# aagbotemi/zk-cryptography

Hardware: AMD Instinct MI355X
Metric: field-evals/s (sumcheck 2^24) + MSM points/s (KZG 2^20) per BASELINE.json; value = the sumcheck prover's field-evals/s, the MSM half is under "msm" (higher is better)
Workload: dtype u32; 1 GPU; 24-var multilinear sumcheck prover (poly_sum + prove), BLS12-381 Fr; field=BLS12-381 Fr (255-bit Montgomery, 8 x u32 limbs); G1 over Fq (381-bit), evals_per_gpu=16777216, exchanges_per_prove=0

## Files before the change

### zk-cryptography_amd/csrc/multifold_kernels.hpp

```cpp
#pragma once
#include "sumcheck_kernels.hpp"
#include "wide_acc.hpp"

namespace zk {

constexpr int MF_MAX_LOGK = 8;
constexpr int MF_CAP_LOGK = 9;

static __global__ __launch_bounds__(MLE_BLOCK) void chunk_sums_kernel(const uint64_t* __restrict__ in, uint32_t chunk,
                                                                      uint64_t* __restrict__ partials) {
    __shared__ Fr red[MLE_BLOCK / 64];
    const uint64_t* base = in + 4 * (size_t)blockIdx.x * chunk;
    Fr s = Fr::zero();
    for (uint32_t j = threadIdx.x; j < chunk; j += 4 * MLE_BLOCK) {
        Fr v[4];
#pragma unroll
        for (int u = 0; u < 4; ++u) v[u] = (j + u * MLE_BLOCK < chunk) ? load_fr(base, j + u * MLE_BLOCK) : Fr::zero();
#pragma unroll
        for (int u = 0; u < 4; ++u) s = s + v[u];
    }
    s = block_reduce_fr(s, red);
    if (threadIdx.x == 0) store_fr(partials, blockIdx.x, s);
}

static __global__ __launch_bounds__(MLE_BLOCK) void group_sums_kernel(const uint64_t* __restrict__ partials, uint32_t group,
                                                                      uint32_t n_blocks, uint64_t* __restrict__ out) {
    __shared__ Fr red[MLE_BLOCK / 64];
    Fr tot = Fr::zero();
    for (uint32_t b = threadIdx.x; b < n_blocks; b += MLE_BLOCK) {
        Fr s = Fr::zero();
        for (uint32_t g = 0; g < group; ++g) s = s + load_fr(partials, (size_t)b * group + g);
        store_fr(out, b, s);
        tot = tot + s;
    }
    tot = block_reduce_fr(tot, red);
    if (threadIdx.x == 0) store_fr(out, n_blocks, tot);
}

constexpr int FINE_CHUNK = 256;
static __global__ __launch_bounds__(MLE_BLOCK) void fine_sums_kernel(const uint64_t* __restrict__ in, size_t n_chunks,
                                                                     uint64_t* __restrict__ sums) {
    const uint32_t lane = threadIdx.x & 63, wave = threadIdx.x >> 6;
    const size_t c0 = ((size_t)blockIdx.x * (MLE_BLOCK / 64) + wave) * 2;
    if (c0 >= n_chunks) return;
    const bool two = c0 + 1 < n_chunks;
    const uint64_t* base = in + 4 * (c0 * FINE_CHUNK);
    Fr v[8];
#pragma unroll
    for (int u = 0; u < 4; ++u) v[u] = load_fr(base, lane + 64 * u);
#pragma unroll
    for (int u = 4; u < 8; ++u) v[u] = two ? load_fr(base, lane + 64 * u) : Fr::zero();
    Fr a = (v[0] + v[1]) + (v[2] + v[3]);
    Fr b = (v[4] + v[5]) + (v[6] + v[7]);
    wave_reduce_fr2(a, b);
    if (lane == 0) {
        store_fr(sums, c0, a);
        if (two) store_fr(sums, c0 + 1, b);
    }
}

static __global__ __launch_bounds__(MLE_BLOCK) void group_sums_wg_kernel(const uint64_t* __restrict__ in, uint32_t group,
                                                                         uint64_t* __restrict__ out_mont, uint64_t* __restrict__ out_canon) {
    __shared__ Fr red[MLE_BLOCK / 64];
    const uint64_t* base = in + 4 * (size_t)blockIdx.x * group;
    Fr s = Fr::zero();
    for (uint32_t j = threadIdx.x; j < group; j += 4 * MLE_BLOCK) {
        Fr v[4];
#pragma unroll
        for (int u = 0; u < 4; ++u) v[u] = (j + u * MLE_BLOCK < group) ? load_fr(base, j + u * MLE_BLOCK) : Fr::zero();
#pragma unroll
        for (int u = 0; u < 4; ++u) s = s + v[u];
    }
    s = block_reduce_fr(s, red);
    if (threadIdx.x == 0) {
        if (out_mont) store_fr(out_mont, blockIdx.x, s);
        if (out_canon) store_fr(out_canon, blockIdx.x, fr_from_mont_outlined(s));
    }
}

constexpr int TREE_MAX_LOG = 10;

struct SmallArgs {
    const uint64_t* src;
    uint32_t group;
    uint32_t stride;
    uint32_t canon;
    uint32_t log_n;
    uint32_t n_rounds;
    uint32_t round0;
    uint32_t first;
    FrArg claimed;
    const uint64_t* d_claimed;
    uint64_t* weights_out;
    uint64_t* final_out;
    long long host_delta;
    uint64_t seq;
    uint64_t* seq_word;
};

constexpr int SMALL_BLOCK = 512;

static __global__ __launch_bounds__(SMALL_BLOCK) void sumcheck_small_kernel(SmallArgs a, SumcheckDev* st,
                                                                            uint64_t* __restrict__ round_polys,
                                                                            uint64_t* __restrict__ challenges) {
    extern __shared__ __attribute__((aligned(16))) unsigned char zk_dyn_lds[];
    __builtin_amdgcn_s_setprio(3);
    ZK_STAMP_AT(0, 40 + a.round0, 0);
    const uint32_t n = 1u << a.log_n;
    Fr* tree0 = reinterpret_cast<Fr*>(zk_dyn_lds);
    Fr* tree1 = tree0 + 2 * n;
    const uint32_t w_all = a.weights_out ? (1u << a.n_rounds) : 0u;
    Fr* w0 = tree1 + n;
    Fr* w1 = w0 + ((a.n_rounds & 1) ? w_all / 2 : w_all);
    const bool grouped = a.group != 0 && a.stride == 0;
    Fr* scratch = w0 + w_all + w_all / 2 + 1;
    Fr* e_sh = scratch + (grouped ? SMALL_BLOCK : 0);
    Fr* r_sh = e_sh + 4;
    if (a.group == 0) {
        for (uint32_t j = threadIdx.x; j < n; j += SMALL_BLOCK) {
            const Fr v = load_fr(a.src, j);
            tree0[n + j] = a.canon ? v : fr_from_mont_outlined(v);
        }
    } else if (a.stride != 0) {
        for (uint32_t j = threadIdx.x; j < n; j += SMALL_BLOCK) {
            Fr s;
            for (uint32_t g = 0; g < a.group; g += 8) {
                Fr v[8];
#pragma unroll
                for (int u = 0; u < 8; ++u) {
                    const uint32_t gu = g + u < a.group ? g + u : a.group - 1;
                    v[u] = load_fr(a.src, (size_t)gu * a.stride + j);
                }
                if (g == 0) s = v[0];
#pragma unroll
                for (int u = 0; u < 8; ++u) if (g + u < a.group && g + u != 0) s = s + v[u];
            }
            tree0[n + j] = a.canon ? s : fr_from_mont_outlined(s);
        }
    } else {
        const uint32_t total = n * a.group;
        const uint32_t run = total > (uint32_t)SMALL_BLOCK ? total / SMALL_BLOCK : 1;
        if (threadIdx.x * run < total) {
            Fr s = Fr::zero();
            for (uint32_t g = 0; g < run; ++g) s = s + load_fr(a.src, (size_t)threadIdx.x * run + g);
            scratch[threadIdx.x] = s;
        }
        __syncthreads();
        const uint32_t tpe = a.group / run;
        for (uint32_t j = threadIdx.x; j < n; j += SMALL_BLOCK) {
            Fr s = scratch[j * tpe];
            for (uint32_t g = 1; g < tpe; ++g) s = s + scratch[j * tpe + g];
            tree0[n + j] = a.canon ? s : fr_from_mont_outlined(s);
        }
    }
    if (threadIdx.x == 0 && a.weights_out) {
        Fr one32;
        constexpr uint32_t c[8] = {0xcaaf6b13u, 0x355094eau, 0x69a568efu, 0xf6b10cb3u, 0x40cc3869u, 0xe2c926a6u, 0xed269aadu, 0x736a6d3bu};
#pragma unroll
        for (int i = 0; i < 8; ++i) one32.l[i] = c[i];
        w0[0] = one32;
    }
    __syncthreads();
    for (uint32_t lvl = a.log_n; lvl > 1;) {
        const uint32_t step = lvl - 1 < 3 ? lvl - 1 : 3;
        const uint32_t groups = 1u << (lvl - step);
        for (uint32_t g = threadIdx.x; g < groups; g += SMALL_BLOCK) {
            Fr v[8];
            const uint32_t cnt0 = 1u << step;
#pragma unroll
            for (int i = 0; i < 8; ++i) if ((uint32_t)i < cnt0) v[i] = tree0[(1u << lvl) + g * cnt0 + i];
#pragma unroll
            for (int sft = 1; sft <= 3; ++sft) {
                if ((uint32_t)sft <= step) {
                    const uint32_t cnt = cnt0 >> sft;
#pragma unroll
                    for (int i = 0; i < 4; ++i) {
                        if ((uint32_t)i < cnt) {
                            v[i] = v[2 * i] + v[2 * i + 1];
                            tree0[(1u << (lvl - sft)) + g * cnt + i] = v[i];
                        }
                    }
                }
            }
        }
        __syncthreads();
        lvl -= step;
    }
    const uint32_t wave = threadIdx.x >> 6;
    const bool wave0 = wave == 0;
    uint32_t* kw1 = reinterpret_cast<uint32_t*>(r_sh + 2);
    uint32_t* kw2 = kw1 + 64;
    uint32_t* dig_sh = kw2 + 64;
    uint32_t* flags = dig_sh + 16;
    if (threadIdx.x >= 64 && threadIdx.x < 66 && a.log_n >= 2)
        e_sh[threadIdx.x - 64] = (tree0[6 + threadIdx.x - 64] - tree0[4 + threadIdx.x - 64]).to_mont();
    if (threadIdx.x == 0) {
        flags[0] = 0; flags[1] = 0;
        uint32_t pre[8];
        if (a.first) {
            const Fr sum_c = (a.first == 2) ? fr_from_mont_outlined(fr_from_arg(a.claimed))
                           : (a.first == 3) ? fr_from_mont_outlined(load_fr(a.d_claimed, 0)) : tree0[2] + tree0[3];
#pragma unroll
            for (int i = 0; i < 8; ++i) pre[i] = sum_c.l[7 - i];
        } else {
#pragma unroll
            for (int i = 0; i < 8; ++i) pre[i] = st->transcript.buf[i];
        }
#pragma unroll
        for (int i = 0; i < 8; ++i) dig_sh[8 + i] = pre[i];
    }
    __syncthreads();
    Fr lo = tree0[2], hi = tree0[3];
    uint32_t depth = a.log_n, round = a.round0, n_w = 1;
    ZK_STAMP_AT(0, 40 + a.round0, 1);
    const uint32_t word = threadIdx.x & 15;
    auto schedule_block1 = [&](const uint32_t* prefix, const Fr& lo_c, uint32_t it) {
        const uint32_t w = word < 8 ? prefix[word] : fr_limb_by_lane(lo_c, 15 - word);
        sha256_schedule_rows_to_lds(w, kw1, flags, 4 * it, 1, threadIdx.x < 64 + 16);
    };
    auto schedule_block2 = [&](const Fr& hi_c, uint32_t it) {
        const uint32_t w = word < 8 ? fr_limb_by_lane(hi_c, 7 - word) : (word == 8 ? 0x80000000u : word == 15 ? 96u * 8u : 0u);
        sha256_schedule_rows_to_lds(w, kw2, flags + 1, 4 * it, 0, threadIdx.x < 128 + 16);
    };
    if (a.n_rounds) {
        if (wave == 1) schedule_block1(dig_sh + 8, lo, 0);
        if (wave == 2) schedule_block2(hi, 0);
    }
    uint32_t digest[8];
    constexpr uint32_t FIRST_HELPER = 192, N_HELPERS = SMALL_BLOCK - FIRST_HELPER - 64, OUT_WAVE = 4;
    if (wave == OUT_WAVE) {
        __builtin_amdgcn_s_setprio(0);
        if (a.host_delta && a.round0) {
            for (uint32_t i = threadIdx.x - 64 * OUT_WAVE; i < 12 * a.round0 + 4; i += 64) {
                const uint64_t* p = i < 4 ? st->sum + i : i < 4 + 8 * a.round0 ? round_polys + (i - 4) : challenges + (i - 4 - 8 * a.round0);
                *const_cast<uint64_t*>(p + a.host_delta) = *p;
            }
        }
    }
    for (uint32_t it = 0; it < a.n_rounds; ++it) {
        Fr* told = (it & 1) ? tree1 : tree0;
        Fr* tnew = (it & 1) ? tree0 : tree1;
        Fr* wold = (it & 1) ? w1 : w0;
        Fr* wnew = (it & 1) ? w0 : w1;
        Fr* eold = e_sh + 2 * (it & 1);
        Fr* enew = e_sh + 2 * ((it & 1) ^ 1);
        const bool absorb_sum = a.first && it == 0;
        if (wave0) {
            ZK_STAMP_AT(0, round, 0);
            uint32_t h[8] = {0x6a09e667u, 0xbb67ae85u, 0x3c6ef372u, 0xa54ff53au, 0x510e527fu, 0x9b05688cu, 0x1f83d9abu, 0x5be0cd19u};
            uint32_t blk[16];
            const uint32_t* pre = dig_sh + 8 * ((it + 1) & 1);
#pragma unroll
            for (int i = 0; i < 8; ++i) { blk[i] = pre[i]; blk[8 + i] = lo.l[7 - i]; }
            ShaSplit sp;
            sp.init();
            uint32_t hs[4];
            sp.split(h, hs);
            sha256_compress_kw_split(sp, hs, blk, kw1, flags, 4 * it);
            ZK_STAMP_AT(0, round, 1);
            sha256_compress_kw_split(sp, hs, nullptr, kw2, flags + 1, 4 * it);
            sp.join(hs, h);
            ZK_STAMP_AT(0, round, 2);
#pragma unroll
            for (int i = 0; i < 8; ++i) digest[i] = h[i];
            Fr c;
#pragma unroll
            for (int i = 0; i < 8; ++i) c.l[i] = h[7 - i];
            c.reduce_once();
            c.reduce_once();
            if (threadIdx.x == 0) {
                r_sh[it & 1] = c;
#pragma unroll
                for (int i = 0; i < 8; ++i) dig_sh[8 * (it & 1) + i] = h[i];
            }
        }
        ZK_STAMP_AT(0, round, 3);
        ZK_STAMP_AT(SMALL_BLOCK - 1, round, 6);
        ZK_STAMP_AT(64, round, 7);
        __syncthreads();
        ZK_STAMP_AT(0, round, 4);
        const Fr c = r_sh[it & 1];
        if (wave0) {
            if (depth >= 2) {
                const uint32_t q = threadIdx.x & 1;
                Fr v = told[4 + q] + fr_mul_outlined(c, eold[q]);
                lo = shfl_fr(v, 0);
                hi = shfl_fr(v, 1);
            }
            ZK_STAMP_AT(0, round, 5);
        } else if (wave <= 2) {
            if (it + 1 < a.n_rounds && depth >= 2) {
                const uint32_t q = wave - 1;
                const Fr v = told[4 + q] + fr_mul_outlined(c, eold[q]);
                if (wave == 1) schedule_block1(dig_sh + 8 * (it & 1), v, it + 1);
                else schedule_block2(v, it + 1);
            }
        } else {
            const Fr r = fr_to_mont_outlined(c);
            const uint32_t helper = wave == OUT_WAVE ? N_HELPERS : wave < OUT_WAVE ? threadIdx.x - FIRST_HELPER : threadIdx.x - FIRST_HELPER - 64;
            if (threadIdx.x == 64 * OUT_WAVE) {
                Fr lo_m = told[2].to_mont(), hi_m = told[3].to_mont();
                if (absorb_sum) {
                    Fr sum_m = (a.first == 2) ? fr_from_arg(a.claimed) : (a.first == 3) ? load_fr(a.d_claimed, 0) : lo_m + hi_m;
                    store_fr(st->sum, 0, sum_m);
                    if (a.host_delta) store_fr(st->sum + a.host_delta, 0, sum_m);
                }
                store_fr(round_polys, 2 * (size_t)round, lo_m);
                store_fr(round_polys, 2 * (size_t)round + 1, hi_m);
                store_fr(challenges, round, r);
                if (a.host_delta) {
                    store_fr(round_polys + a.host_delta, 2 * (size_t)round, lo_m);
                    store_fr(round_polys + a.host_delta, 2 * (size_t)round + 1, hi_m);
                    store_fr(challenges + a.host_delta, round, r);
                }
            }
            const uint32_t nodes = 1u << (depth - 1);
            if (helper >= N_HELPERS - 2 && helper < N_HELPERS && depth >= 3) {
                const uint32_t q = 4 + (helper - (N_HELPERS - 2));
                Fr va = told[q + 4] + r * (told[q + 8] - told[q + 4]);
                Fr vb = told[q + 6] + r * (told[q + 10] - told[q + 6]);
                tnew[q] = va;
                tnew[q + 2] = vb;
                enew[helper - (N_HELPERS - 2)] = (vb - va).to_mont();
            }
            for (uint32_t q = 1 + helper; q < 2 * nodes && helper < N_HELPERS; q += N_HELPERS) {
                if (depth >= 3 && q >= 4 && q < 8) continue;
                const uint32_t p = 1u << (31 - __builtin_clz(q));
                tnew[q] = told[q + p] + r * (told[q + 2 * p] - told[q + p]);
            }
            if (a.weights_out) {
                for (uint32_t b = helper; b < n_w && helper < N_HELPERS; b += N_HELPERS) {
                    Fr w1v = wold[b] * r;
                    wnew[2 * b + 1] = w1v;
                    wnew[2 * b] = wold[b] - w1v;
                }
            }
        }
        n_w <<= 1;
        --depth;
        ++round;
    }
    ZK_STAMP_AT(0, 40 + a.round0, 2);
    if (a.seq_word && wave == OUT_WAVE) __builtin_amdgcn_fence(__ATOMIC_RELEASE, "");
    __syncthreads();
    if (a.seq_word && threadIdx.x == 64 * OUT_WAVE) {
        __hip_atomic_store(a.seq_word, a.seq, __ATOMIC_RELEASE, __HIP_MEMORY_SCOPE_SYSTEM);
        ZK_STAMP_AT(64 * OUT_WAVE, 40 + a.round0, 3);
    }
    if (threadIdx.x == 0 && a.n_rounds) {
        Transcript tr;
        tr.init();
        tr.commit_words8(digest);
        tr.store(&st->transcript);
    }

    if (a.weights_out) {
        Fr* w = (a.n_rounds & 1) ? w1 : w0;
        for (uint32_t b = threadIdx.x; b < n_w; b += SMALL_BLOCK) store_fr(a.weights_out, b, w[b]);
    }
    if (a.final_out) {
        Fr* t = (a.n_rounds & 1) ? tree1 : tree0;
        const uint32_t cnt = 1u << depth;
        for (uint32_t j = threadIdx.x; j < cnt; j += SMALL_BLOCK) store_fr(a.final_out, j, t[cnt + j].to_mont());
    }
}
__host__ __device__ constexpr size_t small_lds_bytes(uint32_t log_n, int weight_rounds, bool grouped) {
    return ((size_t)3 * ((size_t)1 << log_n) + (weight_rounds >= 0 ? 3 * ((size_t)1 << weight_rounds) / 2 : 0u) + 1 +
            (grouped ? SMALL_BLOCK : 0) + 4 + 2) * 32 + (64 + 64 + 16 + 2) * 4;
}

static __global__ __launch_bounds__(MLE_BLOCK) void eq_weights_kernel(PtsArg pts, uint32_t first, uint32_t k,
                                                                      uint64_t* __restrict__ out) {
    const uint32_t b = blockIdx.x * MLE_BLOCK + threadIdx.x;
    if (b >= (1u << k)) return;
    Fr w;
    constexpr uint32_t c[8] = {0xcaaf6b13u, 0x355094eau, 0x69a568efu, 0xf6b10cb3u, 0x40cc3869u, 0xe2c926a6u, 0xed269aadu, 0x736a6d3bu};
#pragma unroll
    for (int i = 0; i < 8; ++i) w.l[i] = c[i];
    const Fr one = Fr::one();
    for (uint32_t i = 0; i < k; ++i) {
        Fr r = fr_from_pts(pts, first + i);
        if (!((b >> (k - 1 - i)) & 1)) r = one - r;
        w = w * r;
    }
    store_fr(out, b, w);
}

static __global__ __launch_bounds__(MLE_BLOCK) void eval_weights_kernel(PtsArg pts, uint32_t k1, uint32_t k2, uint32_t s, uint64_t* __restrict__ w1,
                                                                        uint64_t* __restrict__ wa, uint64_t* __restrict__ wb) {
    size_t b = (size_t)blockIdx.x * MLE_BLOCK + threadIdx.x;
    const size_t n1 = (size_t)1 << k1, na = (size_t)1 << (k2 - s), nb = (size_t)1 << s;
    uint32_t k, first;
    uint64_t* out;
    Fr w = Fr::one();
    if (b < n1) {
        k = k1; first = 0; out = w1;
        constexpr uint32_t c[8] = {0xcaaf6b13u, 0x355094eau, 0x69a568efu, 0xf6b10cb3u, 0x40cc3869u, 0xe2c926a6u, 0xed269aadu, 0x736a6d3bu};
#pragma unroll
        for (int i = 0; i < 8; ++i) w.l[i] = c[i];
    } else if (b < n1 + na) {
        b -= n1; k = k2 - s; first = k1; out = wa;
    } else if (b < n1 + na + nb) {
        b -= n1 + na; k = s; first = k1 + k2 - s; out = wb;
    } else {
        return;
    }
    const Fr one = Fr::one();
    for (uint32_t i = 0; i < k; ++i) {
        Fr r = fr_from_pts(pts, first + i);
        if (!((b >> (k - 1 - i)) & 1)) r = one - r;
        w = w * r;
    }
    store_fr(out, b, w);
}
static __global__ __launch_bounds__(MLE_BLOCK) void sum_records_kernel(const uint64_t* __restrict__ records, uint32_t n, uint64_t* __restrict__ out) {
    __shared__ Fr red[MLE_BLOCK / 64];
    Fr s = Fr::zero();
    for (uint32_t i = threadIdx.x; i < n; i += 4 * MLE_BLOCK) {
        Fr v[4];
#pragma unroll
        for (int u = 0; u < 4; ++u) v[u] = (i + u * MLE_BLOCK < n) ? load_fr(records, i + u * MLE_BLOCK) : Fr::zero();
#pragma unroll
        for (int u = 0; u < 4; ++u) s = s + v[u];
    }
    s = block_reduce_fr(s, red);
    if (threadIdx.x == 0) store_fr(out, 0, s);
}

template <int G, int DEPTH = 4, bool NT = false>
static __global__ __launch_bounds__(1024) void multifold_kernel(const uint64_t* __restrict__ in, size_t m, uint32_t k,
                                                                const uint64_t* __restrict__ weights,
                                                                uint64_t* __restrict__ out,
                                                                uint64_t* __restrict__ partials) {
    constexpr int TG = 64 / G;
    extern __shared__ __attribute__((aligned(16))) unsigned char zk_dyn_lds[];
    Fr* w_lds = reinterpret_cast<Fr*>(zk_dyn_lds);
    Fr* part = w_lds + (1u << k);
    const uint32_t n_terms = 1u << k;
    for (uint32_t b = threadIdx.x; b < n_terms; b += blockDim.x) w_lds[b] = load_fr(weights, b);
    __syncthreads();
    const uint32_t lane = threadIdx.x & 63;
    const uint32_t wave = threadIdx.x >> 6;
    const uint32_t n_waves = blockDim.x >> 6;
    const uint32_t slice = wave * TG + lane / G;
    const uint32_t per = n_terms / (n_waves * TG);
    const uint32_t oj = lane % G;
    const size_t j = (size_t)blockIdx.x * G + oj;
    WideAcc acc;
    acc.clear();
    const uint32_t b0 = slice * per;
    const uint64_t* p = in + 4 * ((size_t)b0 * m + j);
    const size_t row = 4 * m;
    for (uint32_t t = 0; t < per; t += DEPTH) {
        Fr v[DEPTH];
#pragma unroll
        for (int u = 0; u < DEPTH; ++u) if (t + u < per) v[u] = NT ? load_fr_nt(p + (size_t)(t + u) * row) : load_fr(p + (size_t)(t + u) * row, 0);
#pragma unroll
        for (int u = 0; u < DEPTH; ++u) if (t + u < per) acc.mac(w_lds[b0 + t + u], v[u]);
    }
    Fr o = wide_reduce(acc.lo, acc.hi);
#pragma unroll
    for (int d = 32; d >= G; d >>= 1) o = o + shfl_down_fr(o, d);
    if (wave != 0 && lane < G) part[(wave - 1) * G + lane] = o;
    __syncthreads();
    if (wave == 0) {
        if (lane < G) {
            for (uint32_t w2 = 1; w2 < n_waves; ++w2) o = o + part[(w2 - 1) * G + lane];
            store_fr(out, j, o);
        } else {
            o = Fr::zero();
        }
        Fr s = wave_reduce_fr(o);
        if (lane == 0) store_fr(partials, blockIdx.x, s);
    }
}

static __global__ __launch_bounds__(MLE_BLOCK) void slice_sums_kernel(const uint64_t* __restrict__ in, uint32_t ny, uint32_t m,
                                                               uint64_t* __restrict__ out) {
    const uint32_t j = blockIdx.x * MLE_BLOCK + threadIdx.x;
    if (j >= m) return;
    Fr s = load_fr(in, j);
    for (uint32_t y = 1; y < ny; ++y) s = s + load_fr(in, (size_t)y * m + j);
    store_fr(out, j, fr_to_mont_outlined(s));
}

constexpr int BF_BLOCK = 256;
constexpr int BF_LOG_OW = 3;
constexpr int BF_SLICES = BF_BLOCK >> BF_LOG_OW;
constexpr int BF_MAX_PER = 4;
constexpr int BF_MAX_NY = 8;
constexpr int BF_TARGET_WGS = 256;

struct BlockfoldShape { uint32_t log_ow, sl, per, ny; };
__host__ __device__ constexpr bool blockfold_shape(uint32_t m, uint32_t k, BlockfoldShape* sh) {
    if (m == 0 || (m & (m - 1)) != 0 || (m >> BF_LOG_OW) == 0) return false;
    if (k == 0 || k > 10) return false;
    const uint32_t terms = 1u << k, wgx = m >> BF_LOG_OW;
    const uint32_t fill = wgx >= (uint32_t)BF_TARGET_WGS ? 1u : (uint32_t)BF_TARGET_WGS / wgx;
    const uint32_t forced = (terms + BF_SLICES * BF_MAX_PER - 1) / (BF_SLICES * BF_MAX_PER);
    uint32_t ny = fill > forced ? fill : forced;
    if (ny > (uint32_t)BF_MAX_NY) ny = BF_MAX_NY;
    if (ny > terms) ny = terms;
    const uint32_t range = terms / ny;
    sh->log_ow = BF_LOG_OW;
    sh->sl = range < (uint32_t)BF_SLICES ? range : (uint32_t)BF_SLICES;
    sh->per = range / sh->sl;
    sh->ny = ny;
    return true;
}

static __global__ __launch_bounds__(BF_BLOCK) void blockfold_kernel(const uint64_t* __restrict__ in, uint32_t m, uint32_t sl_cnt,
                                                                    uint32_t per, const uint64_t* __restrict__ weights,
                                                                    uint64_t* __restrict__ partial) {
    constexpr uint32_t OW = 1u << BF_LOG_OW, WAVES = BF_BLOCK / 64;
    __shared__ Fr part[(WAVES - 1) * OW];
    const uint32_t lane = threadIdx.x & 63, wave = threadIdx.x >> 6;
    const uint32_t o = lane & (OW - 1), sl = wave * (64 / OW) + (lane >> BF_LOG_OW);
    const uint32_t c = blockIdx.x * OW + o;
    const uint32_t b0 = (blockIdx.y * sl_cnt + sl) * per;
    Fr r = Fr::zero();
    if (sl < sl_cnt) {
        Fr v[BF_MAX_PER], w[BF_MAX_PER];
#pragma unroll
        for (int u = 0; u < BF_MAX_PER; ++u) {
            if ((uint32_t)u < per) { v[u] = load_fr(in, (size_t)(b0 + u) * m + c); w[u] = load_fr(weights, b0 + u); }
        }
        WideAcc acc;
        acc.clear();
#pragma unroll
        for (int u = 0; u < BF_MAX_PER; ++u) {
            if ((uint32_t)u < per) acc.mac(w[u], v[u]);
        }
        r = wide_reduce(acc.lo, acc.hi);
    }
#pragma unroll
    for (int d = 32; d >= (int)OW; d >>= 1) r = r + shfl_down_fr(r, d);
    if (wave != 0 && lane < OW) part[(wave - 1) * OW + lane] = r;
    __syncthreads();
    if (wave == 0 && lane < OW) {
#pragma unroll
        for (uint32_t w2 = 1; w2 < WAVES; ++w2) r = r + part[(w2 - 1) * OW + lane];
        store_fr(partial, (size_t)blockIdx.y * m + c, fr_from_mont_outlined(r));
    }
}

}
```

Before: 56.69 billion field-evals/s.

## Replace per-round challenge multiply with precomputed digit-table affine step in small sumcheck

Inside the fused small sumcheck kernel, the serial critical path (hash, then compute the next round's lo/hi via a full Montgomery multiply by the challenge) is replaced by a table-based affine evaluation. Helper lanes precompute, one round ahead, tables of the coefficient differences times powers of 2^28 in Montgomery form. The critical waves then split the raw hash digest into 28-bit digits and do a row-parallel dot product with DPP carry propagation and ballot-based conditional subtraction. This shortens the latency between hashing and scheduling the next SHA block. The cost is extra LDS, builder work on the last wave, and subtle inline-asm carry logic with some correctness risk.

```diff
diff --git a/zk-cryptography_amd/csrc/affine_step.hpp b/zk-cryptography_amd/csrc/affine_step.hpp
--- /dev/null
+++ b/zk-cryptography_amd/csrc/affine_step.hpp
@@ -0,0 +1,140 @@
+#pragma once
+#include "fp.hpp"
+
+namespace zk {
+
+constexpr int AFF_DIGITS = 10;
+constexpr int AFF_DIGIT_BITS = 28;
+constexpr int AFF_LANE_WORDS = 12;
+constexpr int AFF_TABLE_WORDS = 8 * AFF_LANE_WORDS;
+
+static __constant__ uint32_t AFF_POW_MONT[2 * AFF_DIGITS][8] = {
+    {0xfffffffeu, 0x00000001u, 0x00034802u, 0x5884b7fau, 0xecbc4ff5u, 0x998c4fefu, 0xacc5056fu, 0x1824b159u},
+    {0xdcaaf6b2u, 0x2355094du, 0xa699014eu, 0xf375260du, 0xebe0430au, 0x87cb91f0u, 0x50a25f75u, 0x6567bec7u},
+    {0x120121c9u, 0xebc98da2u, 0x14c66acbu, 0x8676d066u, 0xa9939320u, 0x2382db8fu, 0xdcc56ed3u, 0x3840cb63u},
+    {0x883c74a3u, 0x28e39d79u, 0x9724b837u, 0xfa113d52u, 0xf6f815aeu, 0x2fe69ddbu, 0x2995dcb6u, 0x5c2064bbu},
+    {0x2348f820u, 0xa53acf2au, 0xc830c1b7u, 0x51e1c8bfu, 0x696029a1u, 0x89b7c93du, 0xb9c07cd0u, 0x40ad8d6fu},
+    {0xf712c9b0u, 0xab21c5d1u, 0xb05c2342u, 0xe1e037d0u, 0xc76d0786u, 0x6132d479u, 0x9185dfe8u, 0x1ec1c051u},
+    {0xfbc14b42u, 0x23afe158u, 0x0f78891bu, 0xc839f2f1u, 0x1582b229u, 0x7989f729u, 0x6ed01e4au, 0x22452ae9u},
+    {0x1b4528ecu, 0x9476ebc8u, 0x3fd2a529u, 0x0b3a3b18u, 0xe6447717u, 0xe6670373u, 0xfbd11361u, 0x11c2650fu},
+    {0xbd8c85feu, 0x8427cc90u, 0x0fe630beu, 0xc8ff7852u, 0x27715045u, 0x2b4d2b66u, 0xe5a19691u, 0x05753400u},
+    {0xdf3f29c7u, 0x0c999e98u, 0x4878d702u, 0xf26a5d9du, 0xe8f39c19u, 0x99f809cau, 0x31c3276eu, 0x16311cfdu},
+    {0xf3f29c6du, 0xc999e990u, 0x87925c23u, 0x2b6cedcbu, 0x7254398fu, 0x05d31496u, 0x9f59ff11u, 0x0748d9d9u},
+    {0xcefe9ec4u, 0x10408b02u, 0x81216fd5u, 0x95de93b4u, 0x80951780u, 0x9aa9ea96u, 0xdd800be2u, 0x675f1e93u},
+    {0x31bba87bu, 0x3b344171u, 0x7ede9435u, 0x9902f3d6u, 0x5be041a9u, 0x4fe7f137u, 0xcb4a3990u, 0x412524b5u},
+    {0xa7024848u, 0x1c19723fu, 0x9e1adbcfu, 0x786af0dbu, 0x53ef6d01u, 0x8a7e6bbeu, 0x754967a5u, 0x30cae084u},
+    {0x79440e2cu, 0x012c1658u, 0x513d58f8u, 0xf93e134du, 0xd548296fu, 0x06dfaacdu, 0x6a5a6867u, 0x5f47a474u},
+    {0xb2d98e44u, 0x94bab29eu, 0x9fd1a321u, 0x20f825eeu, 0x2653d3dau, 0x3ccfaa71u, 0x1927907cu, 0x2dcde358u},
+    {0x39ada2e5u, 0xf17ff5ffu, 0x405e5444u, 0x9571c140u, 0x80d885ccu, 0x4503a7fdu, 0x5759c5d6u, 0x661b97c2u},
+    {0x41e84f61u, 0x01b28acdu, 0x3af48bffu, 0xba360e86u, 0xd63f6230u, 0x695b1d64u, 0x1114036du, 0x2d12291au},
+    {0x09c78bb7u, 0xda56f93fu, 0x951b60f5u, 0xa1a23219u, 0x95799a1du, 0x0a05d103u, 0x82e9b152u, 0x55500f41u},
+    {0x6439b73bu, 0xfc62c180u, 0xb8ceec58u, 0xd6efbb11u, 0x9d157cc1u, 0x1a70b147u, 0xcf278b13u, 0x0e218030u}};
+constexpr uint32_t AFF_MU_LO = 0x355094edu;
+constexpr uint64_t AFF_LIMB_LANES = 0x00FF00FF00FF00FFull;
+
+__device__ __forceinline__ Fr affine_pow_mont(uint32_t k) {
+    const uint4* c = reinterpret_cast<const uint4*>(AFF_POW_MONT[k]);
+    const uint4 a = c[0], b = c[1];
+    Fr r;
+    r.l[0] = a.x; r.l[1] = a.y; r.l[2] = a.z; r.l[3] = a.w;
+    r.l[4] = b.x; r.l[5] = b.y; r.l[6] = b.z; r.l[7] = b.w;
+    return r;
+}
+__device__ __forceinline__ void affine_table_store(uint32_t* __restrict__ tbl, uint32_t k, const Fr& tk) {
+#pragma unroll
+    for (int j = 0; j < 8; ++j) tbl[AFF_LANE_WORDS * j + k] = tk.l[j];
+}
+
+__device__ __forceinline__ void affine_digits(const uint32_t (&d)[8], uint32_t (&dg)[AFF_DIGITS]) {
+#pragma unroll
+    for (int k = 0; k < AFF_DIGITS; ++k) {
+        const int w = (AFF_DIGIT_BITS * k) >> 5, s = (AFF_DIGIT_BITS * k) & 31;
+        const uint64_t pair = ((uint64_t)(w + 1 < 8 ? d[w + 1] : 0u) << 32) | d[w];
+        dg[k] = (uint32_t)(pair >> s) & ((1u << AFF_DIGIT_BITS) - 1);
+    }
+}
+
+struct AffineLane {
+    uint32_t p, n;
+    __device__ __forceinline__ void init() {
+        const uint32_t j = threadIdx.x & 15;
+        uint32_t v = 0;
+#pragma unroll
+        for (int i = 0; i < 8; ++i) v = (j == (uint32_t)i) ? FrParams::p(i) : v;
+        p = v;
+        n = j == 0 ? 0u - v : j < 8 ? ~v : 0u;
+    }
+};
+
+template <int CTRL> __device__ __forceinline__ uint32_t aff_dpp0(uint32_t v) {
+    return (uint32_t)__builtin_amdgcn_update_dpp(0, (int)v, CTRL, 0xf, 0xf, true);
+}
+__device__ __forceinline__ uint32_t aff_add_carry(uint32_t w, uint64_t carries) {
+    uint32_t r;
+    asm("v_addc_co_u32 %0, vcc, 0, %1, %2" : "=v"(r) : "v"(w), "s"(carries) : "vcc");
+    return r;
+}
+__device__ __forceinline__ uint32_t aff_sub_borrow(uint32_t a, uint32_t b, uint64_t borrows) {
+    uint32_t r;
+    asm("v_subb_co_u32 %0, vcc, %1, %2, %3" : "=v"(r) : "v"(a), "v"(b), "s"(borrows) : "vcc");
+    return r;
+}
+__device__ __forceinline__ uint32_t aff_select(uint64_t lanes, uint32_t if_set, uint32_t if_clear) {
+    uint32_t r;
+    asm("v_cndmask_b32 %0, %1, %2, %3" : "=v"(r) : "v"(if_clear), "v"(if_set), "s"(lanes));
+    return r;
+}
+__device__ __forceinline__ uint32_t aff_row_mirror(uint32_t v) {
+    uint32_t r;
+    asm("s_nop 1\n\tv_mov_b32_dpp %0, %1 row_mirror row_mask:0xf bank_mask:0xf" : "=v"(r) : "v"(v));
+    return r;
+}
+__device__ __forceinline__ uint32_t aff_row_half_mirror(uint32_t v) {
+    uint32_t r;
+    asm("s_nop 1\n\tv_mov_b32_dpp %0, %1 row_half_mirror row_mask:0xf bank_mask:0xf" : "=v"(r) : "v"(v));
+    return r;
+}
+__device__ __forceinline__ uint64_t aff_carries(uint64_t gen, uint64_t prop) { return ((gen | prop) + gen) ^ prop; }
+
+__device__ __forceinline__ uint32_t affine_step_rows(const AffineLane& c, uint32_t tj, const uint32_t* __restrict__ tbl,
+                                                     const uint32_t (&dg)[AFF_DIGITS]) {
+    constexpr int SHL = 0x100, SHR = 0x110;
+    const uint32_t j = threadIdx.x & 15;
+    uint32_t tk[AFF_LANE_WORDS];
+    uint64_t col = 0;
+    if (j < 8) {
+        const uint4* q = reinterpret_cast<const uint4*>(tbl + AFF_LANE_WORDS * j);
+        const uint4 a = q[0], b = q[1];
+        const uint2 e = *reinterpret_cast<const uint2*>(q + 2);
+        tk[0] = a.x; tk[1] = a.y; tk[2] = a.z; tk[3] = a.w; tk[4] = b.x; tk[5] = b.y; tk[6] = b.z; tk[7] = b.w; tk[8] = e.x; tk[9] = e.y;
+        col = tj;
+#pragma unroll
+        for (int k = 0; k < AFF_DIGITS; ++k) col += (uint64_t)dg[k] * tk[k];
+    }
+    const uint32_t clo = (uint32_t)col, chi = (uint32_t)(col >> 32);
+    const uint32_t hprev = aff_dpp0<SHR + 1>(chi);
+    const uint64_t top = col + hprev;
+    const uint64_t a96 = (uint64_t)(uint32_t)(top >> 32) * AFF_MU_LO + (((uint64_t)(uint32_t)top * AFF_MU_LO) >> 32);
+    uint32_t q = (uint32_t)((a96 + 2 * top) >> 32);
+    q = j == 7 ? q : 0u;
+    q |= aff_dpp0<SHL + 1>(q);
+    q |= aff_dpp0<SHL + 2>(q);
+    q |= aff_dpp0<SHL + 4>(q);
+    const uint64_t g = (uint64_t)q * c.n + clo + hprev;
+    const uint32_t gprev = aff_dpp0<SHR + 1>((uint32_t)(g >> 32));
+    const uint32_t w = (uint32_t)g + gprev;
+    const uint64_t gen = __builtin_amdgcn_ballot_w64(w < gprev);
+    const uint64_t prop = __builtin_amdgcn_ballot_w64(w == 0xFFFFFFFFu) & AFF_LIMB_LANES;
+    uint32_t r = aff_add_carry(w, aff_carries(gen, prop));
+#pragma unroll
+    for (int pass = 0; pass < 2; ++pass) {
+        const uint64_t lt = __builtin_amdgcn_ballot_w64(r < c.p) & AFF_LIMB_LANES;
+        const uint64_t eq = __builtin_amdgcn_ballot_w64(r == c.p) & AFF_LIMB_LANES;
+        const uint64_t bor = aff_carries(lt, eq);
+        const uint64_t below = (bor >> 8) & 0x0001000100010001ull;
+        r = aff_select((below << 8) - below, r, aff_sub_borrow(r, c.p, bor));
+    }
+    return r;
+}
+
+}
diff --git a/zk-cryptography_amd/csrc/multifold_kernels.hpp b/zk-cryptography_amd/csrc/multifold_kernels.hpp
--- a/zk-cryptography_amd/csrc/multifold_kernels.hpp
+++ b/zk-cryptography_amd/csrc/multifold_kernels.hpp
@@ -1,6 +1,7 @@
 #pragma once
 #include "sumcheck_kernels.hpp"
 #include "wide_acc.hpp"
+#include "affine_step.hpp"
 
 namespace zk {
 
@@ -115,7 +116,6 @@
     const bool grouped = a.group != 0 && a.stride == 0;
     Fr* scratch = w0 + w_all + w_all / 2 + 1;
     Fr* e_sh = scratch + (grouped ? SMALL_BLOCK : 0);
-    Fr* r_sh = e_sh + 4;
     if (a.group == 0) {
         for (uint32_t j = threadIdx.x; j < n; j += SMALL_BLOCK) {
             const Fr v = load_fr(a.src, j);
@@ -188,10 +188,12 @@
     }
     const uint32_t wave = threadIdx.x >> 6;
     const bool wave0 = wave == 0;
-    uint32_t* kw1 = reinterpret_cast<uint32_t*>(r_sh + 2);
+    uint32_t* kw1 = reinterpret_cast<uint32_t*>(e_sh + 2);
     uint32_t* kw2 = kw1 + 64;
     uint32_t* dig_sh = kw2 + 64;
     uint32_t* flags = dig_sh + 16;
+    uint32_t* aff_sh = flags + 4;
+    Fr* aff_stage = reinterpret_cast<Fr*>(aff_sh + 4 * AFF_TABLE_WORDS);
     if (threadIdx.x >= 64 && threadIdx.x < 66 && a.log_n >= 2)
         e_sh[threadIdx.x - 64] = (tree0[6 + threadIdx.x - 64] - tree0[4 + threadIdx.x - 64]).to_mont();
     if (threadIdx.x == 0) {
@@ -210,21 +212,33 @@
         for (int i = 0; i < 8; ++i) dig_sh[8 + i] = pre[i];
     }
     __syncthreads();
-    Fr lo = tree0[2], hi = tree0[3];
+    uint32_t low[8];
+#pragma unroll
+    for (int i = 0; i < 8; ++i) low[i] = tree0[2].l[i];
     uint32_t depth = a.log_n, round = a.round0, n_w = 1;
     ZK_STAMP_AT(0, 40 + a.round0, 1);
     const uint32_t word = threadIdx.x & 15;
-    auto schedule_block1 = [&](const uint32_t* prefix, const Fr& lo_c, uint32_t it) {
-        const uint32_t w = word < 8 ? prefix[word] : fr_limb_by_lane(lo_c, 15 - word);
+    auto schedule_block1_words = [&](const uint32_t* prefix, uint32_t lo_w, uint32_t it) {
+        const uint32_t w = word < 8 ? prefix[word] : lo_w;
         sha256_schedule_rows_to_lds(w, kw1, flags, 4 * it, 1, threadIdx.x < 64 + 16);
     };
-    auto schedule_block2 = [&](const Fr& hi_c, uint32_t it) {
-        const uint32_t w = word < 8 ? fr_limb_by_lane(hi_c, 7 - word) : (word == 8 ? 0x80000000u : word == 15 ? 96u * 8u : 0u);
+    auto schedule_block2_words = [&](uint32_t hi_w, uint32_t it) {
+        const uint32_t w = word < 8 ? hi_w : (word == 8 ? 0x80000000u : word == 15 ? 96u * 8u : 0u);
         sha256_schedule_rows_to_lds(w, kw2, flags + 1, 4 * it, 0, threadIdx.x < 128 + 16);
     };
+    auto schedule_block1 = [&](const uint32_t* prefix, const Fr& lo_c, uint32_t it) {
+        schedule_block1_words(prefix, fr_limb_by_lane(lo_c, 15 - word), it);
+    };
+    auto schedule_block2 = [&](const Fr& hi_c, uint32_t it) { schedule_block2_words(fr_limb_by_lane(hi_c, 7 - word), it); };
+    AffineLane aff;
+    aff.init();
+    const uint32_t bl = threadIdx.x - (SMALL_BLOCK - 64);
+    const bool builder = bl < 64 && (bl & 31) < 2 * AFF_DIGITS;
+    const uint32_t b_free = bl >> 5, b_v2 = (bl & 31) >= (uint32_t)AFF_DIGITS ? 1u : 0u, b_k = (bl & 31) - AFF_DIGITS * b_v2;
+    const Fr b_pow = affine_pow_mont(builder ? b_k + AFF_DIGITS * (1 - b_free) : 0u);
     if (a.n_rounds) {
-        if (wave == 1) schedule_block1(dig_sh + 8, lo, 0);
-        if (wave == 2) schedule_block2(hi, 0);
+        if (wave == 1) schedule_block1_words(dig_sh + 8, tree0[2].l[(15 - word) & 7], 0);
+        if (wave == 2) schedule_block2_words(tree0[3].l[(7 - word) & 7], 0);
     }
     uint32_t digest[8];
     constexpr uint32_t FIRST_HELPER = 192, N_HELPERS = SMALL_BLOCK - FIRST_HELPER - 64, OUT_WAVE = 4;
@@ -242,8 +256,9 @@
         Fr* tnew = (it & 1) ? tree0 : tree1;
         Fr* wold = (it & 1) ? w1 : w0;
         Fr* wnew = (it & 1) ? w0 : w1;
-        Fr* eold = e_sh + 2 * (it & 1);
-        Fr* enew = e_sh + 2 * ((it & 1) ^ 1);
+        uint32_t* tbl_old = aff_sh + 2 * AFF_TABLE_WORDS * (it & 1);
+        uint32_t* tbl_new = aff_sh + 2 * AFF_TABLE_WORDS * ((it & 1) ^ 1);
+        const bool tabled = it != 0;
         const bool absorb_sum = a.first && it == 0;
         if (wave0) {
             ZK_STAMP_AT(0, round, 0);
@@ -251,7 +266,7 @@
             uint32_t blk[16];
             const uint32_t* pre = dig_sh + 8 * ((it + 1) & 1);
 #pragma unroll
-            for (int i = 0; i < 8; ++i) { blk[i] = pre[i]; blk[8 + i] = lo.l[7 - i]; }
+            for (int i = 0; i < 8; ++i) { blk[i] = pre[i]; blk[8 + i] = low[7 - i]; }
             ShaSplit sp;
             sp.init();
             uint32_t hs[4];
@@ -263,13 +278,7 @@
             ZK_STAMP_AT(0, round, 2);
 #pragma unroll
             for (int i = 0; i < 8; ++i) digest[i] = h[i];
-            Fr c;
-#pragma unroll
-            for (int i = 0; i < 8; ++i) c.l[i] = h[7 - i];
-            c.reduce_once();
-            c.reduce_once();
             if (threadIdx.x == 0) {
-                r_sh[it & 1] = c;
 #pragma unroll
                 for (int i = 0; i < 8; ++i) dig_sh[8 * (it & 1) + i] = h[i];
             }
@@ -279,52 +288,86 @@
         ZK_STAMP_AT(64, round, 7);
         __syncthreads();
         ZK_STAMP_AT(0, round, 4);
-        const Fr c = r_sh[it & 1];
+        uint32_t dl[8];
         if (wave0) {
-            if (depth >= 2) {
-                const uint32_t q = threadIdx.x & 1;
-                Fr v = told[4 + q] + fr_mul_outlined(c, eold[q]);
-                lo = shfl_fr(v, 0);
-                hi = shfl_fr(v, 1);
-            }
-            ZK_STAMP_AT(0, round, 5);
-        } else if (wave <= 2) {
-            if (it + 1 < a.n_rounds && depth >= 2) {
-                const uint32_t q = wave - 1;
-                const Fr v = told[4 + q] + fr_mul_outlined(c, eold[q]);
-                if (wave == 1) schedule_block1(dig_sh + 8 * (it & 1), v, it + 1);
-                else schedule_block2(v, it + 1);
-            }
+#pragma unroll
+            for (int i = 0; i < 8; ++i) dl[i] = digest[7 - i];
         } else {
-            const Fr r = fr_to_mont_outlined(c);
+#pragma unroll
+            for (int i = 0; i < 8; ++i) dl[i] = dig_sh[8 * (it & 1) + 7 - i];
+        }
+        auto challenge_canonical = [&]() {
+            Fr c;
+#pragma unroll
+            for (int i = 0; i < 8; ++i) c.l[i] = dl[i];
+            c.reduce_once();
+            c.reduce_once();
+            return c;
+        };
+        if (wave <= 2) {
+            const uint32_t q = wave == 2 ? 1u : 0u;
+            if (depth >= 2 && (wave0 || it + 1 < a.n_rounds)) {
+                if (tabled) {
+                    uint32_t dg[AFF_DIGITS];
+                    affine_digits(dl, dg);
+                    const uint32_t limb = affine_step_rows(aff, told[4 + q].l[word & 7], tbl_old + AFF_TABLE_WORDS * q, dg);
+                    if (wave0) {
+#pragma unroll
+                        for (int i = 0; i < 8; ++i) low[i] = __builtin_amdgcn_readlane(limb, i);
+                    } else if (wave == 1) {
+                        schedule_block1_words(dig_sh + 8 * (it & 1), aff_row_mirror(limb), it + 1);
+                    } else {
+                        schedule_block2_words(aff_row_half_mirror(limb), it + 1);
+                    }
+                } else {
+                    const Fr v = told[4 + q] + fr_mul_outlined(challenge_canonical(), e_sh[q]);
+                    if (wave0) {
+#pragma unroll
+                        for (int i = 0; i < 8; ++i) low[i] = v.l[i];
+                    } else {
+                        const Fr vs = v;
+                        if (wave == 1) schedule_block1(dig_sh + 8 * (it & 1), vs, it + 1);
+                        else schedule_block2(vs, it + 1);
+                    }
+                }
+            }
+            if (wave0) ZK_STAMP_AT(0, round, 5);
+        } else {
+            const Fr c = challenge_canonical();
             const uint32_t helper = wave == OUT_WAVE ? N_HELPERS : wave < OUT_WAVE ? threadIdx.x - FIRST_HELPER : threadIdx.x - FIRST_HELPER - 64;
-            if (threadIdx.x == 64 * OUT_WAVE) {
-                Fr lo_m = told[2].to_mont(), hi_m = told[3].to_mont();
+            const uint32_t nodes = 1u << (depth - 1);
+            Fr r = c;
+            if (helper < N_HELPERS && (1 + helper < 2 * nodes || (a.weights_out && helper < n_w))) r = fr_to_mont_outlined(c);
+            if (wave == OUT_WAVE) {
+                const uint32_t ol = threadIdx.x - 64 * OUT_WAVE;
+                Fr m = ol == 1 ? told[2] : ol == 2 ? told[3] : c;
+                if (ol < 3) m = fr_to_mont_outlined(m);
                 if (absorb_sum) {
-                    Fr sum_m = (a.first == 2) ? fr_from_arg(a.claimed) : (a.first == 3) ? load_fr(a.d_claimed, 0) : lo_m + hi_m;
-                    store_fr(st->sum, 0, sum_m);
-                    if (a.host_delta) store_fr(st->sum + a.host_delta, 0, sum_m);
+                    const Fr hi_m = shfl_fr(m, 2);
+                    if (ol == 1) {
+                        Fr sum_m = (a.first == 2) ? fr_from_arg(a.claimed) : (a.first == 3) ? load_fr(a.d_claimed, 0) : m + hi_m;
+                        store_fr(st->sum, 0, sum_m);
+                        if (a.host_delta) store_fr(st->sum + a.host_delta, 0, sum_m);
+                    }
                 }
-                store_fr(round_polys, 2 * (size_t)round, lo_m);
-                store_fr(round_polys, 2 * (size_t)round + 1, hi_m);
-                store_fr(challenges, round, r);
-                if (a.host_delta) {
-                    store_fr(round_polys + a.host_delta, 2 * (size_t)round, lo_m);
-                    store_fr(round_polys + a.host_delta, 2 * (size_t)round + 1, hi_m);
-                    store_fr(challenges + a.host_delta, round, r);
+                if (ol < 3) {
+                    uint64_t* dst = ol == 0 ? challenges + 4 * (size_t)round : round_polys + 4 * (2 * (size_t)round + ol - 1);
+                    store_fr(dst, 0, m);
+                    if (a.host_delta) store_fr(dst + a.host_delta, 0, m);
                 }
             }
-            const uint32_t nodes = 1u << (depth - 1);
-            if (helper >= N_HELPERS - 2 && helper < N_HELPERS && depth >= 3) {
-                const uint32_t q = 4 + (helper - (N_HELPERS - 2));
-                Fr va = told[q + 4] + r * (told[q + 8] - told[q + 4]);
-                Fr vb = told[q + 6] + r * (told[q + 10] - told[q + 6]);
-                tnew[q] = va;
-                tnew[q + 2] = vb;
-                enew[helper - (N_HELPERS - 2)] = (vb - va).to_mont();
+            if (builder && depth >= 3) {
+                const uint32_t q = 4 + b_v2;
+                const Fr x = told[q + 6] - told[q + 4];
+                const Fr y = (told[q + 10] - told[q + 8]) - x;
+                const Fr p1 = (b_free ? x : y) * b_pow;
+                Fr* slot = aff_stage + (bl & 31);
+                if (b_free) *slot = p1;
+                const Fr w = c * p1;
+                __builtin_amdgcn_fence(__ATOMIC_ACQ_REL, "wavefront");
+                if (!b_free) affine_table_store(tbl_new + AFF_TABLE_WORDS * b_v2, b_k, *slot + w);
             }
             for (uint32_t q = 1 + helper; q < 2 * nodes && helper < N_HELPERS; q += N_HELPERS) {
-                if (depth >= 3 && q >= 4 && q < 8) continue;
                 const uint32_t p = 1u << (31 - __builtin_clz(q));
                 tnew[q] = told[q + p] + r * (told[q + 2 * p] - told[q + p]);
             }
@@ -366,7 +409,7 @@
 }
 __host__ __device__ constexpr size_t small_lds_bytes(uint32_t log_n, int weight_rounds, bool grouped) {
     return ((size_t)3 * ((size_t)1 << log_n) + (weight_rounds >= 0 ? 3 * ((size_t)1 << weight_rounds) / 2 : 0u) + 1 +
-            (grouped ? SMALL_BLOCK : 0) + 4 + 2) * 32 + (64 + 64 + 16 + 2) * 4;
+            (grouped ? SMALL_BLOCK : 0) + 2 + 2 * AFF_DIGITS) * 32 + (64 + 64 + 16 + 4 + 4 * AFF_TABLE_WORDS) * 4;
 }
 
 static __global__ __launch_bounds__(MLE_BLOCK) void eq_weights_kernel(PtsArg pts, uint32_t first, uint32_t k,
```

New measurement: 58.78 billion field-evals/s, median of 6. 1.04x the previous value.
